# CenekAlbl/mvus

Measured on AMD Instinct MI355X. Metric: residuals/sec, higher is better.
Workload: dtype f64; 1 GPU; BASELINE configs[2]: 32 cams x 504399 obs (504399 per GPU), rolling shutter on, 5003 spline control points, 15297 params, 1008798 residual rows; step = 1 trust-region trial (residual+Jacobian, LM normal equations + Schur solve, trial residual); solver=lm, parallelism=time-shard x1

## Files before the change

mvus_amd/csrc/ba_api.hip:

```cpp
#include <hip/hip_runtime.h>

#include <algorithm>
#include <atomic>
#include <chrono>
#include <cstring>
#include <dlfcn.h>
#include <map>
#include <mutex>
#include <memory>
#include <string>
#include <vector>

#include "ba_kernels.hip.h"
#include "ba_problem.h"
#include "ba_solver.h"
#include "ba_schur_hip.hip.h"
#include "triangulate.hip.h"
#include "spline_ops.hip.h"
#include "spline_fit.hip.h"
#include "pnp.hip.h"
#include "epipolar.hip.h"

namespace mvus {

// ... 103 lines not shown
    }
    MVUS_HIP(hipGetLastError());
    MVUS_HIP(hipStreamSynchronize(stream));
    m_glob = hp.m;
  }

  ~HipBackend() {
    (void)hipSetDevice(device);
    if (stream) (void)hipStreamSynchronize(stream);
    for (void* p : owned) (void)hipFree(p);
    for (auto& kv : pool_size) (void)hipFree(kv.first);
    if (scal_host) (void)hipHostFree(scal_host);
    if (fetch_ev) (void)hipEventDestroy(fetch_ev);
    for (double* p : sqh_host) if (p) (void)hipHostFree(p);
    if (lsmr_host) (void)hipHostFree(lsmr_host);
    for (int i = 0; i < 2; ++i) if (xmir_host[i]) (void)hipHostFree(xmir_host[i]);
    for (int i = 0; i < kStageSlots; ++i) {
      if (stage[i]) (void)hipHostFree(stage[i]);
      if (stage_ev[i]) (void)hipEventDestroy(stage_ev[i]);
    }
    if (own_stream && stream) (void)hipStreamDestroy(stream);
  }

  int64_t n() const { return hp.n; }
  int64_t m_local() const { return hp.m; }
  int64_t m_global() const { return m_glob; }
  std::map<size_t, std::vector<double*>> pool_free;
  std::map<double*, size_t> pool_size;
  double* alloc(int64_t len) {
    const size_t bytes = (size_t)std::max<int64_t>(len, 1) * sizeof(double);
// ... 173 lines not shown
    if (xmir_cap < hp.n) {
      for (int i = 0; i < 2; ++i) {
        if (xmir_host[i]) { (void)hipHostFree(xmir_host[i]); xmir_host[i] = xmir_dev[i] = nullptr; }
        MVUS_HIP(hipHostMalloc(reinterpret_cast<void**>(&xmir_host[i]), std::max<int64_t>(hp.n, 1) * sizeof(double), hipHostMallocMapped));
        if (hipHostGetDevicePointer(reinterpret_cast<void**>(&xmir_dev[i]), xmir_host[i], 0) != hipSuccess) xmir_dev[i] = nullptr;
      }
      xmir_cap = hp.n;
    }
    return xmir_dev[k];
  }
  const double* mirror_host(int k) const { return scal_direct() ? xmir_host[k] : nullptr; }
  void adopt_residual(double*& f_dev, double*& f_new) {
    if (f_dev == f_cur) f_cur = f_new;
    std::swap(f_dev, f_new);
  }
  void lm_trial(const double* x, const double* p, const double* lb, const double* ub, const double* g, const double* D,
                const int* fail, double* x_new, double* out, double* gnorm_out, double* x_mirror, double* pn2 = nullptr, double delta = 0.0,
                const double* fail_sum = nullptr) {
    touch(x_new);
    double* const fail_out = scal_out() + kFailSumSlot;
    double* pn2_dev = nullptr;
    if (pn2) { if (!tr_pn2) tr_pn2 = dalloc<double>(1); pn2_dev = tr_pn2; dot_into(p, p, hp.n, pn2_dev); }
    const unsigned g2 = hp.n > 2048 && hp.n <= (1 << 17) ? (unsigned)std::min<int64_t>(32, (hp.n + 1023) / 1024) : 0u;
    if (g2 > 1) {
      hipLaunchKernelGGL(k_lm_trial, dim3(g2), dim3(1024), 0, stream, (int)hp.n, x, p, lb, ub, g, D, fail, x_new, out, gnorm_out, partials, (unsigned*)nullptr, x_mirror, (const double*)pn2_dev, delta, fail_sum, fail_out);
      hipLaunchKernelGGL(k_lm_trial_sum, dim3(1), dim3(64), 0, stream, (int)g2, partials, out, gnorm_out, dp, (const double*)x_new, cams);
      cams_for = x_new;
      return;
    }
    hipLaunchKernelGGL(k_lm_trial, dim3(lm_grid()), dim3(1024), 0, stream, (int)hp.n, x, p, lb, ub, g, D, fail, x_new, out, gnorm_out, partials, lm_counter, x_mirror, (const double*)pn2_dev, delta, fail_sum, fail_out);
  }
  void fetch(const double* src, int k, double* host) {
    const int64_t off = src - scal_out();
    const bool queued = fetch_queued && off >= fq_off && off + k <= fq_off + fq_k;
    if (!scal_direct() && !queued) MVUS_HIP(hipMemcpyAsync(scal_host + off, src, sizeof(double) * k, hipMemcpyDeviceToHost, stream));
    fetch_queued = false;
    if (fetch_polled && (scal_direct() || queued)) {
      const volatile double* m = scal_host + kMarkSlot;
      const auto t0 = std::chrono::steady_clock::now();
      unsigned spins = 0;
      while (*m != fetch_seq) {
        if ((++spins & 0xfff) == 0 && std::chrono::steady_clock::now() - t0 > std::chrono::seconds(5)) { MVUS_HIP(hipStreamSynchronize(stream)); break; }
        __builtin_ia32_pause();
      }
      std::atomic_thread_fence(std::memory_order_acquire);
    } else if (fetch_marked && (scal_direct() || queued)) MVUS_HIP(hipEventSynchronize(fetch_ev));
    else MVUS_HIP(hipStreamSynchronize(stream));
    fetch_marked = false; fetch_polled = false;
    for (SqPending& sp : sq_pend)
      if (sp.slot >= off && sp.slot < off + k) { scal_host[sp.slot] = sq_host_sum(sqh_host[&sp - sq_pend], sp.n); sp.slot = -1; }
    for (int i = 0; i < k; ++i) host[i] = scal_host[off + i];
  }
  double dot_n(const double* a, const double* b, int64_t len) { dot_to_slot(a, b, len, 0); return read_slot(0); }
  double dot_m(const double* a, const double* b) { dot_to_slot(a, b, hp.m, 1); reduce(scal_out() + 1, 1); return read_slot(1); }

  void ensure_J() { if (!J) J = dalloc<double>(j_doubles(hp.NS, dp.n_chunks)); }
  void eval(const double* x, double* f, bool jac, int jac_mode) {
    RoctxRange range(jac ? "mvus residual+jacobian" : "mvus residual");
    if (jac) ensure_J();
    const bool masked = jac && jac_mode == MVUS_JAC_PATTERN;
    if (masked && !has_pattern) throw HipError{"MVUS_JAC_PATTERN needs mvus_ba_set_pattern (or solve) first"};
    ensure_cams(x);
    if (dp.n_chunks > 0) {
// ... 85 lines not shown
    if (host_sum) {
      if (need > sqh_cap) {
        for (int i = 0; i < 2; ++i) {
          if (sqh_host[i]) (void)hipHostFree(sqh_host[i]);
          MVUS_HIP(hipHostMalloc(reinterpret_cast<void**>(&sqh_host[i]), need * sizeof(double), hipHostMallocMapped));
          MVUS_HIP(hipHostGetDevicePointer(reinterpret_cast<void**>(&sqh_dev[i]), sqh_host[i], 0));
        }
        sqh_cap = need;
      }
      sq_part = sqh_dev[set];
    } else if (need > sq_cap) { this->sq_part = dalloc<double>(need); sq_cap = need; sq_part = this->sq_part; }
    ensure_cams(x);
    bool cleared = false;
    if (dp.n_chunks > 0) {
      const int fb = (clr && clr_len > 0) ? (int)std::min<int64_t>(2048, (clr_len + kThreads - 1) / kThreads) : 0;
      const dim3 g(dp.n_chunks + fb), b(kThreads);
      double* c = fb > 0 ? clr : (double*)nullptr;
      if (robust()) {
        if (hp.calib) hipLaunchKernelGGL((k_observations<true, false, true>), g, b, 0, stream, dp, cams, x, f, J, rspan, pat0, 0, sq_part, c, (long long)clr_len, loss);
        else hipLaunchKernelGGL((k_observations<false, false, true>), g, b, 0, stream, dp, cams, x, f, J, rspan, pat0, 0, sq_part, c, (long long)clr_len, loss);
      } else {
        if (hp.calib) hipLaunchKernelGGL((k_observations<true, false>), g, b, 0, stream, dp, cams, x, f, J, rspan, pat0, 0, sq_part, c, (long long)clr_len);
        else hipLaunchKernelGGL((k_observations<false, false>), g, b, 0, stream, dp, cams, x, f, J, rspan, pat0, 0, sq_part, c, (long long)clr_len);
      }
      rspan_for = x;
      cleared = fb > 0;
    }
    if (mb > 0 && robust()) hipLaunchKernelGGL((k_motion<false, true>), dim3(mb), dim3(kThreads), 0, stream, dp, x, f + 2 * hp.M, mJ, mctrl, 0, sq_part + dp.n_chunks, loss);
    else if (mb > 0) hipLaunchKernelGGL(k_motion<false>, dim3(mb), dim3(kThreads), 0, stream, dp, x, f + 2 * hp.M, mJ, mctrl, 0, sq_part + dp.n_chunks);
    if (host_sum) { sq_pend[set].slot = out - scal_out(); sq_pend[set].n = dp.n_chunks + mb; }
    else if (dp.n_chunks + mb > 0) hipLaunchKernelGGL(k_dot_final, dim3(1), dim3(kThreads), 0, stream, dp.n_chunks + mb, sq_part, out);
    else MVUS_HIP(hipMemsetAsync(out, 0, sizeof(double), stream));
    reduce(out, 1);
    MVUS_HIP(hipGetLastError());
    return cleared;
  }
  void motion_jacobian(const double* x, double* f) {
    if (hp.T <= 0) return;
// ... 794 lines not shown
      const char* what = opts->solver != MVUS_SOLVER_LM_SCHUR ? "MVUS_SOLVER_TRF_LSMR"
                         : so.jac_mode != MVUS_JAC_ANALYTIC   ? "a Jacobian mode other than MVUS_JAC_ANALYTIC"
                         : (be.allreduce || be.tshard.on)     ? "a sharded handle (set_allreduce / set_rccl / set_time_shard)"
                                                              : nullptr;
      if (what) { be.err = std::string("a robust loss (mvus_ba_set_loss) is not supported with ") + what + ": MVUS_SOLVER_LM_SCHUR with MVUS_JAC_ANALYTIC on one rank only"; return MVUS_E_UNSUPPORTED; }
    }
    if (frozen_on_shards(be, "solve")) return MVUS_E_UNSUPPORTED;
    SolveResult sr;
    be.held_analytic_at_xcur = false;
    if (opts->solver == MVUS_SOLVER_LM_SCHUR) {
      if (be.hp.C * (3 + be.hp.P) > 1152) throw HipError{"LM_SCHUR: reduced camera system larger than 1152 unknowns"};
      if (!h->schur) h->schur.reset(new HipSchur<HipBackend>(be));
      so.lm_lambda0 = be.lm_lambda; so.lm_nu0 = be.lm_nu;
      constexpr double kLambdaMinWide = 0.3;
      if (h->schur->wide && so.lm_trust_radius < 0) so.lm_lambda_min = std::max(so.lm_lambda_min, kLambdaMinWide);
      sr = lm_schur(be, *h->schur, x, lb, ub, so, be.f_cur);
      if (!sr.error) { be.lm_lambda = std::min(std::max(sr.lm_lambda, 1e-12), 1e6); be.lm_nu = std::min(sr.lm_nu, 1024.0); }
      if (sr.jac_stale) be.has_jacobian = false;
    }
    else if (be.frozen_count > 0) {
      struct Flag { bool& f; explicit Flag(bool& b) : f(b) { f = true; } ~Flag() { f = false; } } on(be.freeze_stored_jacobian);
      sr = trf_lsmr(be, xv, lb, ub, so, be.f_cur);
      be.has_jacobian = false;
    }
    else sr = trf_lsmr(be, xv, lb, ub, so, be.f_cur);
    const bool lm = opts->solver == MVUS_SOLVER_LM_SCHUR;
    if (sr.error == -4) {
      MVUS_HIP(hipStreamSynchronize(be.stream));
      h->schur.reset();
      res->cost = sr.cost; res->optimality = 0; res->nfev = sr.nfev; res->njev = sr.njev; res->status = 0; res->lin_iters = sr.lin_iters;
      res->initial_cost = sr.initial_cost; res->solve_ms = std::chrono::duration<double, std::milli>(std::chrono::steady_clock::now() - t0).count();
// ... 1066 lines not shown
```

mvus_amd/csrc/ba_kernels.hip.h:

```cpp
#pragma once
#include <hip/hip_runtime.h>

#include <dlfcn.h>

#include <cstdlib>
#include <string>

#include "ba_math.h"
#include "ba_solver.h"

namespace mvus {

constexpr int kThreads = 256;

struct HipError { std::string msg; int code = -2; };

#define MVUS_HIP(expr)                                                                              \
  do {                                                                                              \
    hipError_t e_ = (expr);                                                                         \
    if (e_ != hipSuccess) throw ::mvus::HipError{std::string(#expr) + ": " + hipGetErrorString(e_)}; \
  } while (0)

struct RoctxApi {
  int (*push)(const char*) = nullptr;
// ... 138 lines not shown
  double *Jx, *Jy;
  long long stride;
  int32_t pat;
  int base;
  bool masked, live;
  int32_t ctrl;
  __device__ __forceinline__ void begin(int32_t c) { ctrl = c; live = !(masked && pat < 0); }
  __device__ __forceinline__ double keep(int k, double v) const {
    return (masked && k >= base && !pattern_has(pat, ctrl + (k - base) / 3)) ? 0.0 : v;
  }
  unsigned lane;
  __device__ __forceinline__ void x(int k, double v) { if (live) MVUS_JSTORE(&(Jx + (long long)k * stride)[lane], keep(k, v)); }
  __device__ __forceinline__ void y(int k, double v) { if (live) MVUS_JSTORE(&(Jy + (long long)k * stride)[lane], keep(k, v)); }
};

template <bool CALIB, bool JAC, bool ROBUST = false, class... L>
__global__ __launch_bounds__(kThreads) __attribute__((amdgpu_waves_per_eu(JAC ? (CALIB ? MVUS_JAC_WAVES_CALIB : MVUS_JAC_WAVES) : 4, 8))) void k_observations(DevProblem dp, const CamState* __restrict__ cams,
                                                           const double* __restrict__ x, double* __restrict__ f,
                                                           double* __restrict__ J, int32_t* __restrict__ span,
                                                           const int32_t* __restrict__ pat0, int masked, double* __restrict__ sq_part = nullptr,
                                                           double* __restrict__ clr = nullptr, long long clr_len = 0, L... loss_v) {
  static_assert(sizeof...(L) == (ROBUST ? 1 : 0), "the robust instantiation is launched with its LossSpec, the linear one without");
  const LossSpec loss = loss_arg(loss_v...);
  constexpr int NS = 3 + (CALIB ? 15 : 6) + 12;
  const int chunk = JAC ? xcd_tile(dp.n_chunks) : (int)blockIdx.x;
  if constexpr (!JAC) {
    if (clr != nullptr && chunk >= dp.n_chunks) {
      const long long nb = (long long)gridDim.x - dp.n_chunks;
      for (long long i = (chunk - dp.n_chunks) * (long long)kThreads + threadIdx.x; i < clr_len; i += nb * kThreads) clr[i] = 0.0;
      return;
    }
  }
  if (chunk >= dp.n_chunks) return;
  const ChunkInfo ci = dp.chunks[chunk];
  const CamState& cam = cams[ci.cam];
  if constexpr (!JAC) {
    if (sq_part != nullptr) {
      __shared__ double sq_red[kThreads / 64];
      double sq = 0.0;
      if ((int)threadIdx.x < ci.count) {
        const long long i = ci.start + threadIdx.x;
        const long long a = ci.cam_start, Mc = ci.cam_count;
        const double uo = CALIB ? 0.0 : dp.u_obs[i], vo = CALIB ? 0.0 : dp.v_obs[i];
// ... 855 lines not shown
  double s[5] = {dead ? __longlong_as_double(0x7ff8000000000000LL) : 0.0, 0.0, 0.0, 0.0, 0.0};
  for (int i0 = blockIdx.x * 1024 + threadIdx.x; i0 < n; i0 += gridDim.x * 1024 * 4) {
    double xv[4], pv[4], gv[4], lo[4], hi[4], dv[4];
#pragma unroll
    for (int u = 0; u < 4; ++u) {
      const int i = i0 + u * gridDim.x * 1024;
      const bool in = i < n;
      xv[u] = in ? x[i] : 0.0; pv[u] = in ? p[i] : 0.0; gv[u] = in ? g[i] : 0.0;
      lo[u] = in ? lb[i] : -INFINITY; hi[u] = in ? ub[i] : INFINITY; dv[u] = in ? D[i] : 0.0;
    }
#pragma unroll
    for (int u = 0; u < 4; ++u) {
      const int i = i0 + u * gridDim.x * 1024;
      if (i >= n) break;
      const double xi = xv[u], pi = pv[u], gi = gv[u];
      const bool ok = isfinite(pi);
      const double xn = (dead || !ok) ? xi : fmin(fmax(xi + cut * pi, lo[u]), hi[u]);
      const double st = xn - xi;
      x_new[i] = xn;
      if (x_mirror) x_mirror[i] = xn;
      s[0] += ok ? gi * st : pi * 0.0; s[1] += st * dv[u] * st; s[2] += st * st; s[3] += xi * xi;
      const bool blocked = (xi <= lo[u] && gi > 0) || (xi >= hi[u] && gi < 0);
      s[4] = fmax(s[4], blocked ? 0.0 : fabs(gi));
    }
  }
#pragma unroll
  for (int k = 0; k < 4; ++k) {
    const double v = wave_sum_dpp(s[k]);
    if ((threadIdx.x & 63) == 0) red[k][threadIdx.x >> 6] = v;
  }
  {
    const double v = wave_max_dpp(s[4]);
    if ((threadIdx.x & 63) == 0) red[4][threadIdx.x >> 6] = v;
  }
  __syncthreads();
  if (threadIdx.x < 5) {
    double t = 0.0;
    for (int w = 0; w < 16; ++w) t = threadIdx.x < 4 ? t + red[threadIdx.x][w] : fmax(t, red[4][w]);
// ... 126 lines not shown
```

mvus_amd/csrc/ba_schur.h:

```cpp
#pragma once
#include <algorithm>
#include <cmath>
#include <cstdio>
#include <limits>
#include <vector>

#include "ba_solver.h"

namespace mvus {

inline double lm_gnorm_host(int64_t n, const double* x, const double* lb, const double* ub, const double* g) {
  double gn = 0;
  for (int64_t i = 0; i < n; ++i) {
    const bool blocked = (x[i] <= lb[i] && g[i] > 0) || (x[i] >= ub[i] && g[i] < 0);
    if (!blocked) gn = std::max(gn, std::fabs(g[i]));
  }
  return gn;
}
inline void lm_trial_host(int64_t n, const double* x, const double* p, const double* lb, const double* ub, const double* g,
                          const double* D, int fail, double* x_new, double* out, double* gnorm_out, double cut = 1.0) {
  double gp = 0, pDp = 0, s2 = 0, x2 = 0;
  bool bad = fail != 0;
  for (int64_t i = 0; i < n && !bad; ++i) bad = !std::isfinite(p[i]);
  for (int64_t i = 0; i < n; ++i) {
    const double xn = bad ? x[i] : std::min(std::max(x[i] + cut * p[i], lb[i]), ub[i]);
    const double st = xn - x[i];
    x_new[i] = xn;
    gp += g[i] * st; pDp += st * D[i] * st; s2 += st * st; x2 += x[i] * x[i];
  }
  out[0] = bad ? std::numeric_limits<double>::quiet_NaN() : gp; out[1] = pDp; out[2] = s2; out[3] = x2;
  *gnorm_out = lm_gnorm_host(n, x, lb, ub, g);
}

template <class B, class Schur>
SolveResult lm_schur(B& be, Schur& sc, double* x, const std::vector<double>& lb, const std::vector<double>& ub,
                     const SolveOptions& opt, double* f_dev) {
  using namespace detail;
  SolveResult res;
  const int64_t n = be.n(), m = be.m_local();
  PoolGuard<B> pool(be);
  int xcur = be.lm_resume(x);
  const bool resumed = xcur >= 0;
  if (!resumed) for (int64_t i = 0; i < n; ++i) if (!(x[i] >= lb[i] && x[i] <= ub[i])) { res.error = -3; return res; }
  if (!resumed) xcur = 0;
  double* x_dev = be.lm_xbuf(xcur);
  double* xt_dev = be.lm_xbuf(xcur ^ 1);
// ... 18 lines not shown
  auto accept_residual = [&] {
    if (B::kSwapResiduals) { double* old = f_new; be.adopt_residual(f_dev, f_new); pool.replace(old, f_new); }
    else be.copy(f_dev, f_new, m);
  };
  int mir_cur = -1, mir_trial = 0;
  bool spec_live = false;
  try {
  const bool tr = opt.lm_trust_radius >= 0;
  double Delta = 0;
  if (tr) {
    Delta = opt.lm_trust_radius;
    if (!(Delta > 0)) { double s2 = 0; for (int64_t i = 0; i < n; ++i) s2 += x[i] * x[i]; Delta = s2 > 0 ? std::sqrt(s2) : 1.0; }
  }
  const int nfetch_all = sc.fail_in_scalars() ? 10 : (tr ? 8 : 7);
  auto launch_trial = [&](double lambda) {
    sc.solve_async(lambda, true);
    be.lm_trial(x_dev, sc.step_ptr(), lbp, ubp, sc.grad_ptr(), sc.diag_ptr(), sc.fail_ptr(), xt_dev, S + 2, S + 1, be.mirror_dev(mir_trial),
                tr ? S + 7 : nullptr, Delta, sc.fail_sum_ptr());
    be.residual_sq(xt_dev, f_new, S + 6);
    spec_live = false;
    if (sc.spec_ok(opt.jac_mode)) { be.fetch_enqueue(S, nfetch_all); sc.linearize_spec(be, xt_dev, f_new, opt.jac_mode); spec_live = true; }
  };
  const int nfetch = nfetch_all;

  double lambda = std::max(opt.lm_lambda0 > 0 ? opt.lm_lambda0 : 1e-4, opt.lm_lambda_min), nu = opt.lm_nu0 > 0 ? opt.lm_nu0 : 2.0;
  const double lambda_min = opt.lm_lambda_min;
  int status = -1;
  double g_norm = 0;
  while (true) {
    const bool can_try = res.nfev < opt.max_nfev;
// ... 172 lines not shown
```

mvus_amd/csrc/ba_schur_hip.hip.h:

```cpp
#pragma once
#include <type_traits>
#include <hip/hip_runtime.h>

#include <algorithm>
#include <cstring>
#include <vector>

#include "ba_kernels.hip.h"
#include "ba_partition.h"
#include "ba_schur.h"

namespace mvus {

constexpr int kNWin = 64;

struct NEView {
  double *A, *gc, *Cb, *gs, *Et;
  double* Apart;
  int C, B, CB, N, N3, W;
  int row0;
  int* err;
};

}
// ... 2141 lines not shown
  }
  const int r = row_lo + blockIdx.x * (kThreads / 64) + (threadIdx.x >> 6);
  if (blockIdx.x == 0 && cams)
    for (int idx = threadIdx.x; idx < ne.CB; idx += kThreads) px[cam_col(dp.C, dp.P, idx / ne.B, idx % ne.B)] = pc[idx];
  if (r >= row_hi) return;
  const double* zr = Z + (long long)r * ncols;
  double acc = 0.0;
  for (int k = lane; k < ne.CB; k += 64) acc += zr[k] * pc[k];
  acc = wave_sum(acc);
  if (lane == 0) {
    const int g = r / 3 + ne.row0, d = r % 3;
    px[dp.mv.ctrl_x0[g] + d * dp.mv.ctrl_stride[g]] = -(acc + zr[ne.CB]);
  }
}

template <int S3>
__global__ __launch_bounds__(256) void k_back_correct(DevProblem dp, NEView ne, PartView pv, int ncols, const double* __restrict__ pc, double* __restrict__ px) {
  const int p = blockIdx.x, i = threadIdx.x;
  constexpr int st = 2 * S3;
  const int r0 = pv.i0[p], nr = pv.i1[p] - r0;
  const int sl = pv.sl[p], sr = pv.sr[p];
  constexpr int nch = 256 / st;
  __shared__ double part[st][nch];
  __shared__ double sx[st];
  double vwv[st];
  const int ic = min(i, max(nr - 1, 0));
  {
    const double* __restrict__ vw = pv.VW + ((long long)p * kPartRowsMax + ic) * st;
#pragma unroll
    for (int a = 0; a < st; ++a) vwv[a] = vw[a];
  }
  const int rrow = r0 + ic, grow = rrow / 3 + ne.row0;
  const int xrow = dp.mv.ctrl_x0[grow] + (rrow % 3) * dp.mv.ctrl_stride[grow];
  const double pold = px[xrow];
  int xsep = 0;
  if (sr >= 0 && i < S3) { const int r = sr + i, g = r / 3 + ne.row0; xsep = dp.mv.ctrl_x0[g] + (r % 3) * dp.mv.ctrl_stride[g]; }
  {
    const int a = i / nch, ch = i - a * nch;
    if (a < st) {
      const bool on = (a < S3 ? sl : sr) >= 0;
      const long long gq = (long long)pv.q_off + p - (a < S3 ? 1 : 0);
      const double* __restrict__ xr = pv.R + ((on ? gq : 0) * S3 + (a % S3)) * ncols;
      double acc = 0.0;
      constexpr int kU = 12;
      for (int k0 = ch; k0 < ne.CB; k0 += nch * kU) {
        double xv[kU], pk[kU];
#pragma unroll
        for (int u = 0; u < kU; ++u) { const int k = min(k0 + nch * u, ne.CB - 1); xv[u] = xr[k]; pk[u] = pc[k]; }
#pragma unroll
        for (int u = 0; u < kU; ++u) acc += k0 + nch * u < ne.CB ? xv[u] * pk[u] : 0.0;
      }
      part[a][ch] = on ? acc : 0.0;
    }
    __syncthreads();
    if (i < st) {
      double t = 0.0;
#pragma unroll
      for (int w = 0; w < nch; ++w) t += part[i][w];
      const bool o = (i < S3 ? sl : sr) >= 0;
      const long long gq = (long long)pv.q_off + p - (i < S3 ? 1 : 0);
      sx[i] = o ? t + pv.R[(gq * S3 + (i % S3)) * ncols + ne.CB] : 0.0;
    }
    __syncthreads();
  }
  if (sr >= 0 && i < S3) px[xsep] = -sx[S3 + i];
  if (i >= nr) return;
  double acc = 0.0;
  if (sl >= 0) {
#pragma unroll
    for (int a = 0; a < S3; ++a) acc += vwv[a] * sx[a];
  }
  if (sr >= 0) {
#pragma unroll
    for (int a = 0; a < S3; ++a) acc += vwv[S3 + a] * sx[S3 + a];
  }
  px[xrow] = pold + acc;
}
static_assert(kPartRowsMax <= 256, "k_back_correct: one thread per row of an interior");

template <class BE>
struct HipSchur {
  BE& be;
  NEView ne{};
  int ncols = 0, BW = 0;
  size_t ne_count = 0;
  double* NEset[2] = {nullptr, nullptr};
  int ne_cur = 0;
  size_t off_gc = 0, off_Cb = 0, off_gs = 0, off_Et = 0, off_Apart = 0;
  double *NE = nullptr, *Lb = nullptr, *Z = nullptr, *G = nullptr, *G0 = nullptr, *S = nullptr, *S2 = nullptr, *Linv = nullptr, *rhs = nullptr, *pc = nullptr,
         *DG = nullptr, *D = nullptr, *gx = nullptr, *px = nullptr, *sepbuf = nullptr;
  RcsView rcs{};
  unsigned* rcs_flags = nullptr;
  bool rcs_trsm_launch = false;
// ... 101 lines not shown
    plan_gemm(3 * (own_hi - own_lo));
    G = be.alloc((size_t)nslab * ne.CB * ncols);
    G0 = be.alloc((size_t)ne.CB * ncols);
    S = be.alloc((size_t)(ne.CB + 1) * ne.CB);
    rhs = be.alloc(ne.CB); pc = be.alloc(ne.CB);
    S2 = be.alloc((size_t)(ne.CB + 1) * ne.CB);
    Linv = be.alloc((size_t)((ne.CB + kNB - 1) / kNB) * kNB * kNB);
    rcs.nn = ne.CB; rcs.nbk = (ne.CB + 15) / 16;
    rcs.Simg = be.alloc(rcs_doubles(ne.CB)); rcs.Tsc = be.alloc(rcs_doubles(ne.CB)); rcs.x = be.alloc((size_t)rcs.nbk * 16);
    MVUS_HIP(hipMalloc(reinterpret_cast<void**>(&rcs_flags), 4 * sizeof(unsigned)));
    MVUS_HIP(hipMemsetAsync(rcs_flags, 0, 4 * sizeof(unsigned), be.stream));
    { const char* e = std::getenv("MVUS_RCS_TRSM"); rcs_trsm_launch = e && std::strcmp(e, "launch") == 0; }
    { const char* e = std::getenv("MVUS_RCS_SPIN_LIMIT"); if (e) rcs_spin_limit = (unsigned)std::strtoul(e, nullptr, 10); }
    { const char* e = std::getenv("MVUS_RCS"); use_rcs = !(e && std::strcmp(e, "gj") == 0); }
    { const char* e = std::getenv("MVUS_BCR_FUSED"); if (e) bcr_fused = std::atoi(e) != 0; }
    MVUS_HIP(hipFuncSetAttribute(reinterpret_cast<const void*>(&k_rcs_trsm), hipFuncAttributeMaxDynamicSharedMemorySize, (int)((rcs_stage_doubles(kRcsSP) + 512) * sizeof(double))));
    MVUS_HIP(hipFuncSetAttribute(reinterpret_cast<const void*>(&k_rcs_backsub), hipFuncAttributeMaxDynamicSharedMemorySize, (int)(rcs_backsub_doubles(rcs.nbk) * sizeof(double))));
    if (shard) { DG = nullptr; D = NE + nAg + halo_count; gx = D + hp.n; }
    else { DG = be.alloc(2 * (size_t)hp.n); D = DG; gx = DG + hp.n; }
    px = be.alloc(hp.n + 2);
    MVUS_HIP(hipMalloc(reinterpret_cast<void**>(&fail), 4 * sizeof(int)));
    MVUS_HIP(hipMemsetAsync(fail, 0, 4 * sizeof(int), be.stream));
    MVUS_HIP(hipHostMalloc(reinterpret_cast<void**>(&fail_host), 2 * sizeof(int), hipHostMallocMapped));
    fail_host[0] = fail_host[1] = 0;
    if (hipHostGetDevicePointer(reinterpret_cast<void**>(&fail_map), fail_host, 0) != hipSuccess) fail_map = nullptr;
    ne.err = fail + 1;
    const bool close = shard && ts.rank + 1 < ts.world;
    part_len = ne.CB <= 128 ? kPartL / 2 : kPartL;
    if (const char* e = std::getenv("MVUS_PART_LEN")) part_len = std::atoi(e);
    const ChainPart cp = partition_chain(own_lo, own_hi - own_lo, sctrl, close, part_len);
// ... 465 lines not shown
      } else {
        hipLaunchKernelGGL(k_sep_factor<S3T>, dim3(1), dim3(64), 0, be.stream, pv, fail);
        hipLaunchKernelGGL(k_sep_rhs<S3T>, dim3((ncols + 63) / 64), dim3(64), 0, be.stream, pv, ncols);
      }
      }
      if (ncorr == 0) {
        const int gy = (ncols + 63) / 64, gz = (kPartRowsMax + kBackRows - 1) / kBackRows;
        const dim3 gback(xcd_grid(pv.P * gy * gz));
        hipLaunchKernelGGL(k_part_back<S3T>, gback, dim3(64), 0, be.stream, pv, ncols, Z, gy, gz);
      }
    }
  }

  bool fail_in_scalars() const { return shard; }
  const double* fail_sum_ptr() const { return shard ? px + be.hp.n : (const double*)nullptr; }
  void solve_async(double lambda, bool trial_follows = false) {
    RoctxRange range("mvus schur solve");
    const long long nLb = (long long)ne.N3 * (BW + 1);
    const long long nZ = (long long)ne.N3 * ncols;
    const int rhs_tiles = (int)((std::max(nZ, nLb) + 255) / 256);
    overlap_chol = std::getenv("MVUS_NO_OVERLAP") == nullptr && !wide;
    if (overlap_chol) {
      const long long nband = std::max<long long>(nLb, (long long)ne.CB + ne.N3);
      hipLaunchKernelGGL(k_band_pack, dim3((unsigned)((nband + 255) / 256)), dim3(256), 0, be.stream, ne, lambda, BW, Lb, fail, be.dp, (int)diag_pending, D, gx);
      rhs_tiles_z = (int)((nZ + 255) / 256);
    } else {
      hipLaunchKernelGGL(k_build_rhs, dim3((unsigned)xcd_grid(rhs_tiles)), dim3(256), 0, be.stream, ne, ncols, Z, (!wide && pv.Dl) ? pv.seprow : (const unsigned char*)nullptr, lambda, BW, Lb, fail, be.dp,
                         (int)diag_pending, D, gx, rhs_tiles);
    }
    diag_pending = false;
    if (wide) {
      const size_t lds_c = (size_t)(BW + 1) * (BW + 1) * sizeof(double), lds_s = (size_t)(BW + 1) * 64 * sizeof(double);
// ... 34 lines not shown
      if (nsp > 1) hipLaunchKernelGGL(k_rcs_backsub, dim3(1), dim3(64 * kRcsBackWaves), rcs_backsub_doubles(nbk) * sizeof(double), be.stream, rcs, pc, nsp - 2);
    } else {
      hipLaunchKernelGGL(k_schur_finish, dim3(ntile, ntile), dim3(kFinThreads), 0, be.stream, ne, ncols, nsl, lambda, Gsum, S, Linv, fail);
      const int nn = ne.CB;
      double* a = S;
      double* b = S2;
      for (int kb = 0; kb < nn; kb += kNB) {
        const int nb = std::min(kNB, nn - kb), below = nn + 1 - (kb + nb);
        const bool last = kb + nb >= nn;
        hipLaunchKernelGGL(k_gj_step, dim3((below + kNB - 1) / kNB, (nn + kNB - 1) / kNB), dim3(kGjThreads), 0, be.stream, nn, kb, a, b, Linv, fail,
                           last ? pc : (double*)nullptr);
        std::swap(a, b);
      }
    }
    const int nrows = row_hi - row_lo, per = kThreads / 64;
    hipLaunchKernelGGL(k_back_substitute, dim3((unsigned)std::max(1, (nrows + per - 1) / per)), dim3(kThreads), 0, be.stream, be.dp, ne, ncols,
                       row_lo, row_hi, (int)(!shard || be.tshard.rank == 0), Z, pc, px, fail, (!shard && be.scal_direct()) ? fail_map : (int*)nullptr,
                       shard ? px + be.hp.n : (double*)nullptr);
    if (!wide && ncorr > 0) {
      if (BW == 11) hipLaunchKernelGGL(k_back_correct<9>, dim3(pv.P), dim3(256), 0, be.stream, be.dp, ne, pv, ncols, (const double*)pc, px);
      else hipLaunchKernelGGL(k_back_correct<15>, dim3(pv.P), dim3(256), 0, be.stream, be.dp, ne, pv, ncols, (const double*)pc, px);
    }
    if (shard) be.reduce(px, (size_t)be.hp.n + 2);
    MVUS_HIP(hipGetLastError());
    if (shard) {
      if (!trial_follows) MVUS_HIP(hipMemcpyAsync(be.scal_host + be.kFailSumSlot, px + be.hp.n, 2 * sizeof(double), hipMemcpyDeviceToHost, be.stream));
    } else if (!be.scal_direct() || !fail_map) MVUS_HIP(hipMemcpyAsync(fail_host, fail, 2 * sizeof(int), hipMemcpyDeviceToHost, be.stream));
  }
};

// ... 24 lines not shown
```

Before: 1.156 billion residuals/s.

## Fuse LM trial step into back-substitution tail and residual kernel front blocks

Measured after the change: 1.182 billion residuals/s, median of 4. About the same (+2.2%).

```diff
diff --git a/mvus_amd/csrc/ba_api.hip b/mvus_amd/csrc/ba_api.hip
--- a/mvus_amd/csrc/ba_api.hip
+++ b/mvus_amd/csrc/ba_api.hip
@@ -141,6 +141,7 @@
     if (fetch_ev) (void)hipEventDestroy(fetch_ev);
     for (double* p : sqh_host) if (p) (void)hipHostFree(p);
     if (lsmr_host) (void)hipHostFree(lsmr_host);
+    if (trial_part_host) (void)hipHostFree(trial_part_host);
     for (int i = 0; i < 2; ++i) if (xmir_host[i]) (void)hipHostFree(xmir_host[i]);
     for (int i = 0; i < kStageSlots; ++i) {
       if (stage[i]) (void)hipHostFree(stage[i]);
@@ -344,9 +345,40 @@
     if (f_dev == f_cur) f_cur = f_new;
     std::swap(f_dev, f_new);
   }
+  const double* tail_done = nullptr;
+  TrialTail trial_tt{};
+  double *trial_part_host = nullptr, *trial_part_dev = nullptr;
+  int64_t trial_out = -1, trial_gnorm = -1;
+  struct TrialPending { int64_t slot = -1, gslot = -1; int groups = 0; } trial_pend;
+  long long tail_fused_count = 0, tail_launch_count = 0;
+  static void trial_host_sum(const double* part, int groups, double* out4, double* gnorm) {
+    double tot[5] = {0.0, 0.0, 0.0, 0.0, 0.0};
+    for (int b = 0; b < groups; ++b)
+      for (int k = 0; k < 5; ++k) {
+        double t = 0.0;
+        for (int w = 0; w < 16; ++w) { const double v = part[(b * 16 + w) * 5 + k]; t = k < 4 ? t + v : std::fmax(t, v); }
+        tot[k] = groups == 1 ? t : (k < 4 ? tot[k] + t : std::fmax(tot[k], t));
+      }
+    for (int k = 0; k < 4; ++k) out4[k] = tot[k];
+    *gnorm = tot[4];
+  }
   void lm_trial(const double* x, const double* p, const double* lb, const double* ub, const double* g, const double* D,
                 const int* fail, double* x_new, double* out, double* gnorm_out, double* x_mirror, double* pn2 = nullptr, double delta = 0.0,
                 const double* fail_sum = nullptr) {
+    if (tail_done != nullptr && tail_done == x_new && pn2 == nullptr && fail_sum == nullptr) {
+      tail_done = nullptr;
+      const int groups = hp.n > 2048 ? (int)std::min<int64_t>(32, (hp.n + 1023) / 1024) : 1;
+      if (!trial_part_host) {
+        MVUS_HIP(hipHostMalloc(reinterpret_cast<void**>(&trial_part_host), 32 * 16 * 5 * sizeof(double), hipHostMallocMapped));
+        MVUS_HIP(hipHostGetDevicePointer(reinterpret_cast<void**>(&trial_part_dev), trial_part_host, 0));
+      }
+      trial_tt = TrialTail{4 * groups, (int)hp.n, groups, x, p, x_new, g, D, lb, ub, fail, x_mirror, trial_part_dev};
+      trial_out = out - scal_out(); trial_gnorm = gnorm_out - scal_out();
+      ++tail_fused_count;
+      return;
+    }
+    tail_done = nullptr;
+    ++tail_launch_count;
     touch(x_new);
     double* const fail_out = scal_out() + kFailSumSlot;
     double* pn2_dev = nullptr;
@@ -377,6 +409,10 @@
     } else if (fetch_marked && (scal_direct() || queued)) MVUS_HIP(hipEventSynchronize(fetch_ev));
     else MVUS_HIP(hipStreamSynchronize(stream));
     fetch_marked = false; fetch_polled = false;
+    if (trial_pend.slot >= off && trial_pend.slot < off + k) {
+      trial_host_sum(trial_part_host, trial_pend.groups, scal_host + trial_pend.slot, scal_host + trial_pend.gslot);
+      trial_pend.slot = -1;
+    }
     for (SqPending& sp : sq_pend)
       if (sp.slot >= off && sp.slot < off + k) { scal_host[sp.slot] = sq_host_sum(sqh_host[&sp - sq_pend], sp.n); sp.slot = -1; }
     for (int i = 0; i < k; ++i) host[i] = scal_host[off + i];
@@ -492,14 +528,16 @@
     bool cleared = false;
     if (dp.n_chunks > 0) {
       const int fb = (clr && clr_len > 0) ? (int)std::min<int64_t>(2048, (clr_len + kThreads - 1) / kThreads) : 0;
-      const dim3 g(dp.n_chunks + fb), b(kThreads);
+      TrialTail tt{};
+      if (trial_tt.nfront > 0 && trial_tt.x_new == x) { tt = trial_tt; trial_tt.nfront = 0; trial_pend.slot = trial_out; trial_pend.gslot = trial_gnorm; trial_pend.groups = tt.groups; }
+      const dim3 g(tt.nfront + dp.n_chunks + fb), b(kThreads);
       double* c = fb > 0 ? clr : (double*)nullptr;
       if (robust()) {
-        if (hp.calib) hipLaunchKernelGGL((k_observations<true, false, true>), g, b, 0, stream, dp, cams, x, f, J, rspan, pat0, 0, sq_part, c, (long long)clr_len, loss);
-        else hipLaunchKernelGGL((k_observations<false, false, true>), g, b, 0, stream, dp, cams, x, f, J, rspan, pat0, 0, sq_part, c, (long long)clr_len, loss);
+        if (hp.calib) hipLaunchKernelGGL((k_observations<true, false, true>), g, b, 0, stream, dp, cams, x, f, J, rspan, pat0, 0, sq_part, c, (long long)clr_len, tt, loss);
+        else hipLaunchKernelGGL((k_observations<false, false, true>), g, b, 0, stream, dp, cams, x, f, J, rspan, pat0, 0, sq_part, c, (long long)clr_len, tt, loss);
       } else {
-        if (hp.calib) hipLaunchKernelGGL((k_observations<true, false>), g, b, 0, stream, dp, cams, x, f, J, rspan, pat0, 0, sq_part, c, (long long)clr_len);
-        else hipLaunchKernelGGL((k_observations<false, false>), g, b, 0, stream, dp, cams, x, f, J, rspan, pat0, 0, sq_part, c, (long long)clr_len);
+        if (hp.calib) hipLaunchKernelGGL((k_observations<true, false>), g, b, 0, stream, dp, cams, x, f, J, rspan, pat0, 0, sq_part, c, (long long)clr_len, tt);
+        else hipLaunchKernelGGL((k_observations<false, false>), g, b, 0, stream, dp, cams, x, f, J, rspan, pat0, 0, sq_part, c, (long long)clr_len, tt);
       }
       rspan_for = x;
       cleared = fb > 0;
@@ -1324,7 +1362,9 @@
       so.lm_lambda0 = be.lm_lambda; so.lm_nu0 = be.lm_nu;
       constexpr double kLambdaMinWide = 0.3;
       if (h->schur->wide && so.lm_trust_radius < 0) so.lm_lambda_min = std::max(so.lm_lambda_min, kLambdaMinWide);
+      const long long tf0 = be.tail_fused_count, tl0 = be.tail_launch_count;
       sr = lm_schur(be, *h->schur, x, lb, ub, so, be.f_cur);
+      if (std::getenv("MVUS_DEBUG")) std::fprintf(stderr, "lm tail: %lld trials fused, %lld by launches\n", be.tail_fused_count - tf0, be.tail_launch_count - tl0);
       if (!sr.error) { be.lm_lambda = std::min(std::max(sr.lm_lambda, 1e-12), 1e6); be.lm_nu = std::min(sr.lm_nu, 1024.0); }
       if (sr.jac_stale) be.has_jacobian = false;
     }
diff --git a/mvus_amd/csrc/ba_kernels.hip.h b/mvus_amd/csrc/ba_kernels.hip.h
--- a/mvus_amd/csrc/ba_kernels.hip.h
+++ b/mvus_amd/csrc/ba_kernels.hip.h
@@ -176,19 +176,69 @@
   __device__ __forceinline__ void y(int k, double v) { if (live) MVUS_JSTORE(&(Jy + (long long)k * stride)[lane], keep(k, v)); }
 };
 
+__device__ __forceinline__ double lm_trial_point(double x, double p, double lo, double hi, bool dead, double cut) {
+  return (dead || !isfinite(p)) ? x : fmin(fmax(x + cut * p, lo), hi);
+}
+__device__ __forceinline__ void lm_trial_terms(double (&s)[5], double xi, double pi, double gi, double lo, double hi, double dv, double xn) {
+  const bool ok = isfinite(pi);
+  const double st = xn - xi;
+  s[0] += ok ? gi * st : pi * 0.0; s[1] += st * dv * st; s[2] += st * st; s[3] += xi * xi;
+  const bool blocked = (xi <= lo && gi > 0) || (xi >= hi && gi < 0);
+  s[4] = fmax(s[4], blocked ? 0.0 : fabs(gi));
+}
+struct TrialTail {
+  int nfront = 0, n = 0, groups = 0;
+  const double *x = nullptr, *p = nullptr, *x_new = nullptr, *g = nullptr, *D = nullptr, *lb = nullptr, *ub = nullptr;
+  const int* fail = nullptr;
+  double *x_mirror = nullptr, *part = nullptr;
+};
+__device__ __forceinline__ void lm_trial_front(const TrialTail& t) {
+  const int group = (int)blockIdx.x >> 2, tid = (((int)blockIdx.x & 3) << 8) | (int)threadIdx.x;
+  const bool dead = t.fail[0] != 0;
+  double s[5] = {dead ? __longlong_as_double(0x7ff8000000000000LL) : 0.0, 0.0, 0.0, 0.0, 0.0};
+  for (int i0 = group * 1024 + tid; i0 < t.n; i0 += t.groups * 1024 * 4) {
+    double xv[4], pv[4], gv[4], lo[4], hi[4], dv[4], xn[4];
+#pragma unroll
+    for (int u = 0; u < 4; ++u) {
+      const int i = i0 + u * t.groups * 1024;
+      const bool in = i < t.n;
+      xv[u] = in ? t.x[i] : 0.0; pv[u] = in ? t.p[i] : 0.0; gv[u] = in ? t.g[i] : 0.0; xn[u] = in ? t.x_new[i] : 0.0;
+      lo[u] = in ? t.lb[i] : -INFINITY; hi[u] = in ? t.ub[i] : INFINITY; dv[u] = in ? t.D[i] : 0.0;
+    }
+#pragma unroll
+    for (int u = 0; u < 4; ++u) {
+      const int i = i0 + u * t.groups * 1024;
+      if (i >= t.n) break;
+      if (t.x_mirror) t.x_mirror[i] = xn[u];
+      lm_trial_terms(s, xv[u], pv[u], gv[u], lo[u], hi[u], dv[u], xn[u]);
+    }
+  }
+  double* const out = t.part + (long long)(group * 16 + (tid >> 6)) * 5;
+#pragma unroll
+  for (int k = 0; k < 4; ++k) {
+    const double v = wave_sum_dpp(s[k]);
+    if ((threadIdx.x & 63) == 0) out[k] = v;
+  }
+  {
+    const double v = wave_max_dpp(s[4]);
+    if ((threadIdx.x & 63) == 0) out[4] = v;
+  }
+}
+
 template <bool CALIB, bool JAC, bool ROBUST = false, class... L>
 __global__ __launch_bounds__(kThreads) __attribute__((amdgpu_waves_per_eu(JAC ? (CALIB ? MVUS_JAC_WAVES_CALIB : MVUS_JAC_WAVES) : 4, 8))) void k_observations(DevProblem dp, const CamState* __restrict__ cams,
                                                            const double* __restrict__ x, double* __restrict__ f,
                                                            double* __restrict__ J, int32_t* __restrict__ span,
                                                            const int32_t* __restrict__ pat0, int masked, double* __restrict__ sq_part = nullptr,
-                                                           double* __restrict__ clr = nullptr, long long clr_len = 0, L... loss_v) {
+                                                           double* __restrict__ clr = nullptr, long long clr_len = 0, TrialTail tt = TrialTail{}, L... loss_v) {
   static_assert(sizeof...(L) == (ROBUST ? 1 : 0), "the robust instantiation is launched with its LossSpec, the linear one without");
   const LossSpec loss = loss_arg(loss_v...);
   constexpr int NS = 3 + (CALIB ? 15 : 6) + 12;
-  const int chunk = JAC ? xcd_tile(dp.n_chunks) : (int)blockIdx.x;
+  const int chunk = JAC ? xcd_tile(dp.n_chunks) : (int)blockIdx.x - tt.nfront;
   if constexpr (!JAC) {
+    if (chunk < 0) { lm_trial_front(tt); return; }
     if (clr != nullptr && chunk >= dp.n_chunks) {
-      const long long nb = (long long)gridDim.x - dp.n_chunks;
+      const long long nb = (long long)gridDim.x - tt.nfront - dp.n_chunks;
       for (long long i = (chunk - dp.n_chunks) * (long long)kThreads + threadIdx.x; i < clr_len; i += nb * kThreads) clr[i] = 0.0;
       return;
     }
@@ -1074,14 +1124,10 @@
       const int i = i0 + u * gridDim.x * 1024;
       if (i >= n) break;
       const double xi = xv[u], pi = pv[u], gi = gv[u];
-      const bool ok = isfinite(pi);
-      const double xn = (dead || !ok) ? xi : fmin(fmax(xi + cut * pi, lo[u]), hi[u]);
-      const double st = xn - xi;
+      const double xn = lm_trial_point(xi, pi, lo[u], hi[u], dead, cut);
       x_new[i] = xn;
       if (x_mirror) x_mirror[i] = xn;
-      s[0] += ok ? gi * st : pi * 0.0; s[1] += st * dv[u] * st; s[2] += st * st; s[3] += xi * xi;
-      const bool blocked = (xi <= lo[u] && gi > 0) || (xi >= hi[u] && gi < 0);
-      s[4] = fmax(s[4], blocked ? 0.0 : fabs(gi));
+      lm_trial_terms(s, xi, pi, gi, lo[u], hi[u], dv[u], xn);
     }
   }
 #pragma unroll
diff --git a/mvus_amd/csrc/ba_schur.h b/mvus_amd/csrc/ba_schur.h
--- a/mvus_amd/csrc/ba_schur.h
+++ b/mvus_amd/csrc/ba_schur.h
@@ -30,6 +30,15 @@
   }
   out[0] = bad ? std::numeric_limits<double>::quiet_NaN() : gp; out[1] = pDp; out[2] = s2; out[3] = x2;
   *gnorm_out = lm_gnorm_host(n, x, lb, ub, g);
+}
+
+namespace detail {
+template <class Schur>
+auto plan_tail(Schur& sc, const double* x, const double* lb, const double* ub, double* x_new, int) -> decltype(sc.plan_tail(x, lb, ub, x_new), void()) {
+  sc.plan_tail(x, lb, ub, x_new);
+}
+template <class Schur>
+void plan_tail(Schur&, const double*, const double*, const double*, double*, long) {}
 }
 
 template <class B, class Schur>
@@ -78,6 +87,7 @@
   }
   const int nfetch_all = sc.fail_in_scalars() ? 10 : (tr ? 8 : 7);
   auto launch_trial = [&](double lambda) {
+    if (!tr) detail::plan_tail(sc, x_dev, lbp, ubp, xt_dev, 0);
     sc.solve_async(lambda, true);
     be.lm_trial(x_dev, sc.step_ptr(), lbp, ubp, sc.grad_ptr(), sc.diag_ptr(), sc.fail_ptr(), xt_dev, S + 2, S + 1, be.mirror_dev(mir_trial),
                 tr ? S + 7 : nullptr, Delta, sc.fail_sum_ptr());
diff --git a/mvus_amd/csrc/ba_schur_hip.hip.h b/mvus_amd/csrc/ba_schur_hip.hip.h
--- a/mvus_amd/csrc/ba_schur_hip.hip.h
+++ b/mvus_amd/csrc/ba_schur_hip.hip.h
@@ -2179,6 +2179,54 @@
   }
 }
 
+template <int S3, int kU = 12>
+__device__ __forceinline__ void sep_partials(const NEView& ne, const PartView& pv, int ncols, int p, int sl, int sr, const double* __restrict__ pc,
+                                             double (*part)[256 / (2 * S3)]) {
+  constexpr int st = 2 * S3, nch = 256 / st;
+  const int i = threadIdx.x;
+  const int a = i / nch, ch = i - a * nch;
+  if (a < st) {
+    const bool on = (a < S3 ? sl : sr) >= 0;
+    const long long gq = (long long)pv.q_off + p - (a < S3 ? 1 : 0);
+    const double* __restrict__ xr = pv.R + ((on ? gq : 0) * S3 + (a % S3)) * ncols;
+    double acc = 0.0;
+    for (int k0 = ch; k0 < ne.CB; k0 += nch * kU) {
+      double xv[kU], pk[kU];
+#pragma unroll
+      for (int u = 0; u < kU; ++u) { const int k = min(k0 + nch * u, ne.CB - 1); xv[u] = xr[k]; pk[u] = pc[k]; }
+#pragma unroll
+      for (int u = 0; u < kU; ++u) acc += k0 + nch * u < ne.CB ? xv[u] * pk[u] : 0.0;
+    }
+    part[a][ch] = on ? acc : 0.0;
+  }
+}
+template <int S3>
+__device__ __forceinline__ void sep_sums(const NEView& ne, const PartView& pv, int ncols, int p, int sl, int sr, const double (*part)[256 / (2 * S3)],
+                                         double* sx) {
+  constexpr int st = 2 * S3, nch = 256 / st;
+  const int i = threadIdx.x;
+  if (i < st) {
+    double t = 0.0;
+#pragma unroll
+    for (int w = 0; w < nch; ++w) t += part[i][w];
+    const bool o = (i < S3 ? sl : sr) >= 0;
+    const long long gq = (long long)pv.q_off + p - (i < S3 ? 1 : 0);
+    sx[i] = o ? t + pv.R[(gq * S3 + (i % S3)) * ncols + ne.CB] : 0.0;
+  }
+}
+template <int S3>
+__device__ __forceinline__ double sep_correction(const double (&vwv)[2 * S3], const double* sx, int sl, int sr) {
+  double acc = 0.0;
+  if (sl >= 0) {
+#pragma unroll
+    for (int a = 0; a < S3; ++a) acc += vwv[a] * sx[a];
+  }
+  if (sr >= 0) {
+#pragma unroll
+    for (int a = 0; a < S3; ++a) acc += vwv[S3 + a] * sx[S3 + a];
+  }
+  return acc;
+}
 template <int S3>
 __global__ __launch_bounds__(256) void k_back_correct(DevProblem dp, NEView ne, PartView pv, int ncols, const double* __restrict__ pc, double* __restrict__ px) {
   const int p = blockIdx.x, i = threadIdx.x;
@@ -2200,48 +2248,106 @@
   const double pold = px[xrow];
   int xsep = 0;
   if (sr >= 0 && i < S3) { const int r = sr + i, g = r / 3 + ne.row0; xsep = dp.mv.ctrl_x0[g] + (r % 3) * dp.mv.ctrl_stride[g]; }
-  {
-    const int a = i / nch, ch = i - a * nch;
-    if (a < st) {
-      const bool on = (a < S3 ? sl : sr) >= 0;
-      const long long gq = (long long)pv.q_off + p - (a < S3 ? 1 : 0);
-      const double* __restrict__ xr = pv.R + ((on ? gq : 0) * S3 + (a % S3)) * ncols;
-      double acc = 0.0;
-      constexpr int kU = 12;
-      for (int k0 = ch; k0 < ne.CB; k0 += nch * kU) {
-        double xv[kU], pk[kU];
-#pragma unroll
-        for (int u = 0; u < kU; ++u) { const int k = min(k0 + nch * u, ne.CB - 1); xv[u] = xr[k]; pk[u] = pc[k]; }
-#pragma unroll
-        for (int u = 0; u < kU; ++u) acc += k0 + nch * u < ne.CB ? xv[u] * pk[u] : 0.0;
-      }
-      part[a][ch] = on ? acc : 0.0;
-    }
-    __syncthreads();
-    if (i < st) {
-      double t = 0.0;
-#pragma unroll
-      for (int w = 0; w < nch; ++w) t += part[i][w];
-      const bool o = (i < S3 ? sl : sr) >= 0;
-      const long long gq = (long long)pv.q_off + p - (i < S3 ? 1 : 0);
-      sx[i] = o ? t + pv.R[(gq * S3 + (i % S3)) * ncols + ne.CB] : 0.0;
-    }
-    __syncthreads();
-  }
+  sep_partials<S3>(ne, pv, ncols, p, sl, sr, pc, part);
+  __syncthreads();
+  sep_sums<S3>(ne, pv, ncols, p, sl, sr, part, sx);
+  __syncthreads();
   if (sr >= 0 && i < S3) px[xsep] = -sx[S3 + i];
   if (i >= nr) return;
-  double acc = 0.0;
-  if (sl >= 0) {
-#pragma unroll
-    for (int a = 0; a < S3; ++a) acc += vwv[a] * sx[a];
-  }
-  if (sr >= 0) {
-#pragma unroll
-    for (int a = 0; a < S3; ++a) acc += vwv[S3 + a] * sx[S3 + a];
-  }
-  px[xrow] = pold + acc;
+  px[xrow] = pold + sep_correction<S3>(vwv, sx, sl, sr);
 }
 static_assert(kPartRowsMax <= 256, "k_back_correct: one thread per row of an interior");
+
+template <int S3>
+__global__ __launch_bounds__(256, S3 == 9 ? 4 : 3) void k_step_tail(DevProblem dp, NEView ne, PartView pv, int ncols, int nsl, const double* __restrict__ Z,
+                                                   const double* __restrict__ pc, double* __restrict__ px, int* fail, int* __restrict__ fail_mirror,
+                                                   const double* __restrict__ x, const double* __restrict__ lb, const double* __restrict__ ub,
+                                                   double* __restrict__ x_new, CamState* __restrict__ cams) {
+  extern __shared__ double tail_head[];
+  constexpr int st = 2 * S3, nch = 256 / st;
+  __shared__ double part[st][nch];
+  __shared__ double sx[st];
+  __shared__ double prow[kPartRowsMax];
+  const int p = (int)blockIdx.x / nsl, slice = (int)blockIdx.x - p * nsl, i = threadIdx.x;
+  const int f0 = fail[0], f2 = fail[2];
+  const bool dead = f0 != 0 || f2 != 0;
+  const int r0 = pv.i0[p], nr = pv.i1[p] - r0;
+  const int sl = pv.sl[p], sr = pv.sr[p];
+  const int per = (nr + nsl - 1) / nsl, lo = min(slice * per, nr), cnt = min(per, nr - lo);
+  double vwv[st];
+  const int ic = min(lo + min(i, max(cnt - 1, 0)), max(nr - 1, 0));
+  {
+    const double* __restrict__ vw = pv.VW + ((long long)p * kPartRowsMax + ic) * st;
+#pragma unroll
+    for (int a = 0; a < st; ++a) vwv[a] = vw[a];
+  }
+  const int rrow = r0 + ic, grow = rrow / 3 + ne.row0;
+  const int xrow = dp.mv.ctrl_x0[grow] + (rrow % 3) * dp.mv.ctrl_stride[grow];
+  const double xr_x = x[xrow], xr_lo = lb[xrow], xr_hi = ub[xrow];
+  const bool sep_thread = slice == 0 && sr >= 0 && i < S3;
+  int xsep = 0;
+  if (sep_thread) { const int r = sr + i, g = r / 3 + ne.row0; xsep = dp.mv.ctrl_x0[g] + (r % 3) * dp.mv.ctrl_stride[g]; }
+  if (blockIdx.x == 0) {
+    if (i < 2) {
+      int v = i == 0 ? f0 : fail[1];
+      if (i == 0 && f2 != 0) { v = kFailHandoverCode; fail[0] = v; }
+      if (fail_mirror != nullptr) fail_mirror[i] = v;
+    }
+    for (int idx = i; idx < ne.CB; idx += 256) {
+      const int col = cam_col(dp.C, dp.P, idx / ne.B, idx % ne.B);
+      const double v = pc[idx];
+      const double xn = lm_trial_point(x[col], v, lb[col], ub[col], dead, 1.0);
+      px[col] = v; x_new[col] = xn; tail_head[col] = xn;
+    }
+  }
+  sep_partials<S3, 6>(ne, pv, ncols, p, sl, sr, pc, part);
+  {
+    const int wave = i >> 6, lane = i & 63;
+    constexpr int RB = 5;
+    const int q = (cnt + 3) / 4, jend = min(cnt, (wave + 1) * q);
+    for (int j0 = wave * q; j0 < jend; j0 += RB) {
+      const double* zr[RB];
+      double acc[RB];
+#pragma unroll
+      for (int u = 0; u < RB; ++u) { zr[u] = Z + (long long)(r0 + lo + min(j0 + u, jend - 1)) * ncols; acc[u] = 0.0; }
+      for (int k = lane; k < ne.CB; k += 128) {
+        const int k2 = min(k + 64, ne.CB - 1);
+        const bool on2 = k + 64 < ne.CB;
+        double z1[RB], z2[RB];
+#pragma unroll
+        for (int u = 0; u < RB; ++u) { z1[u] = zr[u][k]; z2[u] = zr[u][k2]; }
+        const double p1 = pc[k], p2 = pc[k2];
+#pragma unroll
+        for (int u = 0; u < RB; ++u) {
+          acc[u] += z1[u] * p1;
+          if (on2) acc[u] += z2[u] * p2;
+        }
+      }
+#pragma unroll
+      for (int u = 0; u < RB; ++u) {
+        const double t = wave_sum(acc[u]);
+        if (lane == 0 && j0 + u < jend) prow[j0 + u] = -(t + zr[u][ne.CB]);
+      }
+    }
+  }
+  __syncthreads();
+  sep_sums<S3>(ne, pv, ncols, p, sl, sr, part, sx);
+  __syncthreads();
+  if (sep_thread) {
+    const double v = -sx[S3 + i];
+    px[xsep] = v; x_new[xsep] = lm_trial_point(x[xsep], v, lb[xsep], ub[xsep], dead, 1.0);
+  }
+  if (i < cnt) {
+    const double v = prow[i] + sep_correction<S3>(vwv, sx, sl, sr);
+    px[xrow] = v; x_new[xrow] = lm_trial_point(xr_x, v, xr_lo, xr_hi, dead, 1.0);
+  }
+  if (blockIdx.x != 0) return;
+  for (int c = i; c < dp.C; c += 256) {
+    CamState cs;
+    load_cam_state(tail_head, dp.C, c, dp.calib != 0, dp.Kfix, dp.dfix, dp.H[c], cs);
+    cams[c] = cs;
+  }
+}
 
 template <class BE>
 struct HipSchur {
@@ -2373,6 +2479,7 @@
     { const char* e = std::getenv("MVUS_RCS_SPIN_LIMIT"); if (e) rcs_spin_limit = (unsigned)std::strtoul(e, nullptr, 10); }
     { const char* e = std::getenv("MVUS_RCS"); use_rcs = !(e && std::strcmp(e, "gj") == 0); }
     { const char* e = std::getenv("MVUS_BCR_FUSED"); if (e) bcr_fused = std::atoi(e) != 0; }
+    { const char* e = std::getenv("MVUS_LM_TAIL"); tail_fused = !(e && std::strcmp(e, "launches") == 0); }
     MVUS_HIP(hipFuncSetAttribute(reinterpret_cast<const void*>(&k_rcs_trsm), hipFuncAttributeMaxDynamicSharedMemorySize, (int)((rcs_stage_doubles(kRcsSP) + 512) * sizeof(double))));
     MVUS_HIP(hipFuncSetAttribute(reinterpret_cast<const void*>(&k_rcs_backsub), hipFuncAttributeMaxDynamicSharedMemorySize, (int)(rcs_backsub_doubles(rcs.nbk) * sizeof(double))));
     if (shard) { DG = nullptr; D = NE + nAg + halo_count; gx = D + hp.n; }
@@ -2868,8 +2975,16 @@
 
   bool fail_in_scalars() const { return shard; }
   const double* fail_sum_ptr() const { return shard ? px + be.hp.n : (const double*)nullptr; }
+  const double *tail_x = nullptr, *tail_lb = nullptr, *tail_ub = nullptr;
+  double* tail_xnew = nullptr;
+  bool tail_armed = false;
+  bool tail_fused = true;
+  void plan_tail(const double* x, const double* lb, const double* ub, double* x_new) {
+    tail_x = x; tail_lb = lb; tail_ub = ub; tail_xnew = x_new; tail_armed = true;
+  }
   void solve_async(double lambda, bool trial_follows = false) {
     RoctxRange range("mvus schur solve");
+    be.tail_done = nullptr;
     const long long nLb = (long long)ne.N3 * (BW + 1);
     const long long nZ = (long long)ne.N3 * ncols;
     const int rhs_tiles = (int)((std::max(nZ, nLb) + 255) / 256);
@@ -2934,6 +3049,22 @@
       }
     }
     const int nrows = row_hi - row_lo, per = kThreads / 64;
+    const bool tail = trial_follows && tail_armed && tail_fused && !shard && !wide && ncorr > 0 && be.scal_direct() && fail_map != nullptr &&
+                      be.hp.n <= (1 << 17) && be.dp.n_chunks > 0;
+    tail_armed = false;
+    if (tail) {
+      const int nsl = std::min(16, std::max(1, 1024 / pv.P));
+      const size_t lds = (size_t)ne.CB * sizeof(double);
+      be.touch(tail_xnew);
+      if (BW == 11) hipLaunchKernelGGL(k_step_tail<9>, dim3((unsigned)(pv.P * nsl)), dim3(256), lds, be.stream, be.dp, ne, pv, ncols, nsl, (const double*)Z, (const double*)pc, px,
+                                       fail, fail_map, tail_x, tail_lb, tail_ub, tail_xnew, be.cams);
+      else hipLaunchKernelGGL(k_step_tail<15>, dim3((unsigned)(pv.P * nsl)), dim3(256), lds, be.stream, be.dp, ne, pv, ncols, nsl, (const double*)Z, (const double*)pc, px,
+                              fail, fail_map, tail_x, tail_lb, tail_ub, tail_xnew, be.cams);
+      be.cams_for = tail_xnew;
+      be.tail_done = tail_xnew;
+      MVUS_HIP(hipGetLastError());
+      return;
+    }
     hipLaunchKernelGGL(k_back_substitute, dim3((unsigned)std::max(1, (nrows + per - 1) / per)), dim3(kThreads), 0, be.stream, be.dp, ne, ncols,
                        row_lo, row_hi, (int)(!shard || be.tshard.rank == 0), Z, pc, px, fail, (!shard && be.scal_direct()) ? fail_map : (int*)nullptr,
                        shard ? px + be.hp.n : (double*)nullptr);
```
